# KaffinPX/neptune-core

Measured on AMD Instinct MI355X. Metric: STARK proofs verified/sec (whole node) + Tip5 perms/sec vs VALU roofline, higher is better.
Workload: dtype u64 (Goldilocks mod p; XFE = cubic extension)

## Files before the change

neptune-core_amd/csrc/stark_kernels.hip:

```cpp
#include <hip/hip_ext.h>

#include <atomic>
#include <cstdlib>

#include "../../include/nhip_challenge_id.h"
#include "kernels.hpp"
#include "proof_codec.hpp"
#include "stark.hpp"
#include "tip5_device.hpp"
#include "xfe.hpp"

namespace nhip {

#ifndef NHIP_LAT_PRIO
#define NHIP_LAT_PRIO 2
#endif
__device__ __forceinline__ void latency_priority() {
    if constexpr (NHIP_LAT_PRIO > 0) __builtin_amdgcn_s_setprio(NHIP_LAT_PRIO);
}
static constexpr uint32_t AGE_PRIO_OLDEST = 2;
static constexpr uint32_t AGE_PRIO_MIN_PROOFS = 2048;
__device__ uint32_t g_batches_done;
struct AgePrio {
    uint32_t seq, k;
};
__device__ __forceinline__ void age_priority(AgePrio a, int base) {
    bool old = false;
    if (a.k) {
        const uint32_t done = __builtin_amdgcn_readfirstlane(
            __hip_atomic_load(&g_batches_done, __ATOMIC_RELAXED, __HIP_MEMORY_SCOPE_AGENT));
        old = (int32_t)(a.seq - done) < (int32_t)a.k;
    }
    switch (base + (old ? 1 : 0)) {
        case 0: break;
        case 1: __builtin_amdgcn_s_setprio(1); break;
        case 2: __builtin_amdgcn_s_setprio(2); break;
        default: __builtin_amdgcn_s_setprio(3); break;
    }
}
#ifndef NHIP_MP_PRIO
#define NHIP_MP_PRIO 1
#endif


template <bool MW>
__device__ __forceinline__ Xfe ld_xfe_w(const uint64_t* __restrict__ w, uint64_t off) {
    return {word_mont<MW>(w[off]), word_mont<MW>(w[off + 1]), word_mont<MW>(w[off + 2])};
}
__device__ __forceinline__ Xfe ld_xfe_raw(const uint64_t* __restrict__ w, uint64_t off) {
    return {w[off], w[off + 1], w[off + 2]};
}
__device__ __forceinline__ void st_xfe_raw(uint64_t* __restrict__ w, uint64_t off, Xfe v) {
    w[off] = v.c0;
    w[off + 1] = v.c1;
    w[off + 2] = v.c2;
}
__device__ __forceinline__ bool x_is_zero(Xfe a) { return (a.c0 | a.c1 | a.c2) == 0; }

__device__ __forceinline__ uint64_t root_of_unity(uint32_t log2n) {
    return b_pow(to_mont(7), (GL_P - 1) >> log2n);
}

template <bool MW>
__global__ void __launch_bounds__(64) k_decode(const uint64_t* __restrict__ words, const ProofIn* __restrict__ in,
                                               uint32_t n_proofs, Dims D, uint32_t fs_stride, uint32_t xs_stride,
                                               ProofDesc* __restrict__ desc, FsOp* __restrict__ ops,
                                               uint32_t* __restrict__ fail, unsigned long long* __restrict__ counters) {
    latency_priority();
    __shared__ ProofDesc spd;
    __shared__ uint32_t sfail;
    __shared__ int sdeg;
    const uint32_t p = blockIdx.x, lane = threadIdx.x;
    if (p >= n_proofs) return;
    const ProofIn pin = in[p];
    if (lane == 0) {
        uint64_t perms = 0, perms_lcw = 0;
        const ClaimLoc cl{pin.claim_off, pin.claim_in_n, pin.claim_out_n};
        uint32_t f = decode_stream<MW>(words, pin.off, pin.len, cl, D, spd, ops + (uint64_t)p * fs_stride, perms, perms_lcw);
        if (!f && spd.log2_ph != pin.sized_log2_ph) {
            f = FAIL_DECODE;
            spd = ProofDesc{};
            claim_offsets(spd, cl);
        }
        if (!f) {
            atomicAdd(counters + CNT_PERMS_STATIC, (unsigned long long)perms);
            atomicAdd(counters + CNT_PERMS_LCW, (unsigned long long)perms_lcw);
        }
        sfail = f;
        sdeg = -1;
    }
    __syncthreads();
    const uint32_t f = sfail;
    if (!f) {
        int deg = -1;
        for (uint32_t hi = spd.last_poly_n; hi > 0; hi = hi > 64 ? hi - 64 : 0) {
            bool nz = false;
            if (lane < hi) {
                const uint64_t* x = words + spd.last_poly_off + 3ull * (hi - 1 - lane);
                nz = (canon(x[0]) | canon(x[1]) | canon(x[2])) != 0;
            }
            const uint64_t b = __ballot(nz);
            if (b) {
                deg = (int)(hi - (uint32_t)__ffsll((unsigned long long)b));
                break;
            }
        }
        if (lane == 0) sdeg = deg;
    }
    __syncthreads();
    if (lane == 0) {
        if (!f) last_poly_finish(spd, sdeg, D);
        const SampleLayout sl = SampleLayout::of(D.d, spd.R);
        spd.fs_op_off = p * fs_stride;
        spd.xs_off = (uint64_t)p * xs_stride;
        spd.n_xs = f ? 0u : sl.total;
        spd.idx_off = (uint64_t)p * D.d.num_checks;
        fail[p] = f;
    }
    __syncthreads();
    const uint64_t* src = reinterpret_cast<const uint64_t*>(&spd);
    uint64_t* dst = reinterpret_cast<uint64_t*>(desc + p);
    for (uint32_t i = lane; i < sizeof(ProofDesc) / 8; i += 64) dst[i] = src[i];
}

template <bool PAIR, bool MW>
__device__ __forceinline__ void fs_replay_wide_body(uint32_t bx, const Tip5Lds& lds, const uint64_t* __restrict__ words,
                                                    const ProofDesc* __restrict__ desc,
                                                    const FsOp* __restrict__ ops, uint32_t n_proofs,
                                                    uint64_t* __restrict__ xs, uint32_t* __restrict__ idx_out,
                                                    const uint32_t* __restrict__ fail) {
    constexpr uint32_t LANES = PAIR ? 32u : 16u;
    const uint32_t e = threadIdx.x & 15u;
    const uint32_t h = PAIR ? (threadIdx.x >> 4) & 1u : 0u;
    const uint32_t g = (bx * blockDim.x + threadIdx.x) / LANES;
    if (g >= n_proofs || fail[g]) return;
    uint64_t rc[TIP5_ROUNDS];
#pragma unroll
    for (int r = 0; r < TIP5_ROUNDS; ++r) rc[r] = c_tip5_rc_raw[r * 16 + e];
    uint32_t cm[8];
#pragma unroll
    for (int j = 0; j < 8; ++j) cm[j] = h ? TIP5_MDS[j + 8] : TIP5_MDS[j];
    auto permute = [&](uint64_t st) {
        if constexpr (PAIR) return tip5_permute_pair(st, e, h, rc, cm, lds.lut);
        else return tip5_permute_wide<false>(st, e, rc, lds.lut);
    };
    const bool writer = h == 0;
    const ProofDesc& d = desc[g];
    uint64_t s = 0;
    uint64_t xcur = d.xs_off * 3;
    uint64_t icur = d.idx_off;
    const uint32_t row_shift = threadIdx.x & (64u - LANES);
    for (uint32_t o = 0; o < d.fs_op_n; ++o) {
        const FsOp op = ops[d.fs_op_off + o];
        if (op.kind == FS_ABSORB) {
            const uint64_t* __restrict__ src = words + op.arg;
            const uint32_t len = op.n;
            const uint32_t nchunks = len / TIP5_RATE + 1;
            uint64_t w = (e < TIP5_RATE && e < len) ? src[e] : 0ull;
// ... 941 lines not shown
        const Xfe except_last = x_sub(z, x_lift(w_inv));
        const Xfe zm1 = x_sub(z, x_one());
        Xfe zph = z;
        for (uint32_t q = 0; q < d.log2_ph; ++q) zph = x_mul(zph, zph);
        const Xfe cons = x_sub(zph, x_one());
        const bool z0 = x_is_zero(zm1), z1 = x_is_zero(cons), z3 = x_is_zero(except_last);
        if (z0 || z1 || z3) zero_flag = 1u;
        const Xfe a = z0 ? x_one() : zm1, b = z1 ? x_one() : cons, c = z3 ? x_one() : except_last;
        const Xfe ab = x_mul(a, b);
        const Xfe iabc = x_inv(x_mul(ab, c));
        const Xfe iab = x_mul(iabc, c);
        const Xfe i1 = z1 ? x_zero() : x_mul(iab, a);
        zinv[0] = z0 ? x_zero() : x_mul(iab, b);
        zinv[1] = i1;
        zinv[2] = x_mul(except_last, i1);
        zinv[3] = z3 ? x_zero() : x_mul(iabc, ab);
    } else if (tid >= 64 && tid < 256) {
        auto chal = [&](uint32_t i) { return ld_xfe_raw(xs, xb + 3ull * (sl.chal + i)); };
        const uint32_t wv = tid >> 6;
        if (wv == 1) {
            const Xfe lut = eval_terminal_wave(256u, chal(CH_LOOKUP_TABLE_PUBLIC), [&](uint32_t i) {
                const uint64_t y = i + 1;
                return to_mont((y * y % 257u * y % 257u + 256u) % 257u);
            });
            if (tid == 64) chal_derived[2] = lut;
        } else if (wv == 2) {
            const Xfe ein = eval_terminal_wave(d.claim_in_n, chal(CH_STANDARD_INPUT),
                                               [&](uint32_t i) { return word_mont<MW>(words[d.claim_in_off + i]); });
            const Xfe comp = eval_terminal_wave(5u, chal(CH_COMPRESS_PROGRAM_DIGEST),
                                                [&](uint32_t i) { return word_mont<MW>(words[d.claim_digest_off + i]); });
            if (tid == 128) {
                chal_derived[0] = ein;
                chal_derived[3] = comp;
            }
        } else {
            const Xfe eout = eval_terminal_wave(d.claim_out_n, chal(CH_STANDARD_OUTPUT),
                                                [&](uint32_t i) { return word_mont<MW>(words[d.claim_out_off + i]); });
            if (tid == 192) chal_derived[1] = eout;
        }
    }
    __syncthreads();
    const uint32_t offs[5] = {0u, cons_type_off.x, cons_type_off.y, cons_type_off.z, cons_type_off.w};
    auto fetch = [&](uint32_t ref) -> Xfe {
        const uint32_t t = ref >> 30;
        if (t == 0) return slot_ld(ref);
        if (t == 1) return consts[ref & 0x3FFFFFFFu];
        const uint32_t kind = (ref >> 27) & 7u, i = ref & 0x7FFFFFFu;
        switch (kind) {
            case IN_MAIN_CURR: return ld_xfe_w<MW>(words, d.ood_mc + 3ull * i);
            case IN_AUX_CURR: return ld_xfe_w<MW>(words, d.ood_ac + 3ull * i);
            case IN_MAIN_NEXT: return ld_xfe_w<MW>(words, d.ood_mn + 3ull * i);
            case IN_AUX_NEXT: return ld_xfe_w<MW>(words, d.ood_an + 3ull * i);
            default:
                return i < dims.num_sampled ? ld_xfe_raw(xs, xb + 3ull * (sl.chal + i)) : chal_derived[i - dims.num_sampled];
        }
    };
    for (uint32_t lvl = 0; lvl < n_levels; ++lvl) {
        const uint32_t s0 = seg_off[3 * lvl], s1 = seg_off[3 * lvl + 1], s2 = seg_off[3 * lvl + 2],
                       s3 = seg_off[3 * lvl + 3];
        for (uint32_t q = s0 + tid; q < s1; q += blockDim.x) {
            const uint4 ins = reinterpret_cast<const uint4*>(prog)[q];
            slot_st(ins.w, fetch(ins.y));
        }
        for (uint32_t q = s1 + tid; q < s2; q += blockDim.x) {
            const uint4 ins = reinterpret_cast<const uint4*>(prog)[q];
            slot_st(ins.w, x_mul(slot_ld(ins.y), slot_ld(ins.z)));
        }
        for (uint32_t q = s2 + tid; q < s3; q += blockDim.x) {
            const uint4 ins = reinterpret_cast<const uint4*>(prog)[q];
            const Xfe x = slot_ld(ins.y), y = slot_ld(ins.z);
            slot_st(ins.w, ins.x == OOD_ADD ? x_add(x, y) : x_sub(x, y));
        }
        __syncthreads();
    }
    const uint32_t C = dims.num_constraints, cbase = lds_slots + gslot_n - C;
    Xfe acc = x_zero();
    for (uint32_t c = tid; c < C; c += blockDim.x) {
        uint32_t t = 0;
        while (t < 3 && c >= offs[t + 1]) ++t;
        const Xfe w = ld_xfe_raw(xs, xb + 3ull * (sl.quot_w + c));
        acc = x_add(acc, x_mul(w, x_mul(slot_ld(cbase + c), zinv[t])));
    }
    const Xfe ood_q = block_sum_xfe_waves(acc, red);
    const uint32_t M = dims.num_main, A = dims.num_aux, Q = dims.num_quot_seg;
    Xfe lc = x_zero(), ln = x_zero();
    for (uint32_t c = tid; c < M + A; c += blockDim.x) {
        const Xfe w = ld_xfe_raw(xs, xb + 3ull * (sl.lin_w + c));
        const Xfe vc = c < M ? ld_xfe_w<MW>(words, d.ood_mc + 3ull * c) : ld_xfe_w<MW>(words, d.ood_ac + 3ull * (c - M));
        const Xfe vn = c < M ? ld_xfe_w<MW>(words, d.ood_mn + 3ull * c) : ld_xfe_w<MW>(words, d.ood_an + 3ull * (c - M));
        lc = x_add(lc, x_mul(w, vc));
        ln = x_add(ln, x_mul(w, vn));
    }
    const Xfe sum_c = block_sum_xfe_waves(lc, red);
    const Xfe sum_n = block_sum_xfe_waves(ln, red);
    if (tid >= 64) return;
    Xfe seg = x_zero(), qlin = x_zero();
    for (uint32_t base = 0; base < Q; base += 64u) {
        const uint32_t q = base + tid, top = min(Q - 1u, base + 63u);
        Xfe zk = (q & 1u) ? z : x_one(), zp = z;
        for (uint32_t e = top >> 1, bit = 1; e; e >>= 1, ++bit) {
            zp = x_mul(zp, zp);
            zk = x_mul(zk, ((q >> bit) & 1u) ? zp : x_one());
        }
        if (q < Q) {
            const Xfe sq = ld_xfe_w<MW>(words, d.ood_qs + 3ull * q);
            seg = x_add(seg, x_mul(zk, sq));
            qlin = x_add(qlin, x_mul(ld_xfe_raw(xs, xb + 3ull * (sl.lin_w + M + A + q)), sq));
        }
    }
#pragma unroll
    for (int m = 32; m > 0; m >>= 1) {
        seg = x_add(seg, shfl_xor_xfe(seg, m));
        qlin = x_add(qlin, shfl_xor_xfe(qlin, m));
    }
    if (tid == 0) {
        uint32_t f = 0;
        if (zero_flag) f |= FAIL_ZERO_INVERSE;
        if (!x_eq(seg, ood_q)) f |= FAIL_OOD;
        if (f) atomicOr(&fail[p], f);
        uint64_t* o = ood_out + (uint64_t)p * 9;
        st_xfe_raw(o, 0, sum_c);
        st_xfe_raw(o, 3, sum_n);
        st_xfe_raw(o, 6, qlin);
    }
}

__device__ __forceinline__ uint64_t lds_pow(const uint64_t* __restrict__ sq, uint64_t e) {
    uint64_t r = MONT_ONE;
    for (uint32_t b = 0; e; ++b, e >>= 1)
        if (e & 1) r = mont_mul(r, sq[b]);
    return r;
}

#ifndef NHIP_FRI_WAVES
#define NHIP_FRI_WAVES 1
#endif
template <bool MW>
__device__ __forceinline__ void fri_body(uint32_t p, const uint64_t* __restrict__ words, const ProofDesc* __restrict__ desc,
                                         uint32_t n_proofs, StarkDims dims, const uint64_t* __restrict__ xs,
                                         const uint32_t* __restrict__ idx_all, uint64_t* __restrict__ xdom,
                                         uint32_t* __restrict__ fail) {
    __shared__ Xfe red[256];
    __shared__ uint64_t gsq[33], wsq[33];
    __shared__ uint32_t lflag;
    const uint32_t tid = threadIdx.x;
    if (p >= n_proofs || (fail[p] & FAIL_DECODE)) return;
    const ProofDesc& d = desc[p];
    const SampleLayout sl = SampleLayout::of(dims, d.R);
    const uint64_t xb = d.xs_off * 3;
    const uint32_t k = dims.num_checks;
    const uint32_t* __restrict__ idx = idx_all + d.idx_off;
    const uint32_t L = d.last_cw_n;
    const uint32_t log2L = 31 - __clz(L);
    if (tid == 0) {
        lflag = 0;
        uint64_t g = root_of_unity(d.log2_N);
        for (uint32_t q = 0; q < d.log2_N; ++q, g = mont_mul(g, g)) gsq[q] = g;
    } else if (tid == 64) {
        uint64_t w = root_of_unity(log2L);
        for (uint32_t q = 0; q < log2L; ++q, w = mont_mul(w, w)) wsq[q] = w;
    }
    __syncthreads();
    uint32_t f = 0;
    if (tid < k) {
        const uint32_t i0 = idx[tid];
        Xfe a = ld_xfe_w<MW>(words, d.fri[0].leaves_off + 3ull * tid);
        uint64_t x = mont_mul(to_mont(7), lds_pow(gsq, i0));
        xdom[(uint64_t)p * k + tid] = x;
        uint64_t xinv = b_inv(x);
        const uint64_t neg_half = to_mont((GL_P - 1) / 2);
        for (uint32_t r = 0; r < d.R; ++r) {
            const Xfe b = ld_xfe_w<MW>(words, d.fri[1 + r].leaves_off + 3ull * tid);
            const Xfe alpha = ld_xfe_raw(xs, xb + 3ull * (sl.alpha + r));
            const Xfe slope = x_scale(x_sub(b, a), mont_mul(neg_half, xinv));
            a = x_add(a, x_mul(slope, x_sub(alpha, x_lift(x))));
            x = mont_mul(x, x);
            xinv = mont_mul(xinv, xinv);
        }
        const Xfe last = ld_xfe_w<MW>(words, d.last_cw_off + 3ull * (i0 & (L - 1)));
        if (!x_eq(last, a)) f |= FAIL_FRI_LAST_AGREE;
    }
    const Xfe t = ld_xfe_raw(xs, xb + 3ull * sl.indeterminate);
    Xfe num = x_zero(), den = x_zero();
    if (tid < L) {
        uint64_t wi = lds_pow(wsq, tid);
        const uint64_t wstep = blockDim.x < L ? wsq[31 - __clz(blockDim.x)] : MONT_ONE;
        auto term = [&](uint32_t i, uint64_t w, Xfe inv) {
            const Xfe q = x_scale(inv, w);
            num = x_add(num, x_mul(q, ld_xfe_w<MW>(words, d.last_cw_off + 3ull * i)));
            den = x_add(den, q);
        };
        uint32_t i = tid;
        for (; i + blockDim.x < L; i += 2 * blockDim.x) {
            const uint64_t w1 = mont_mul(wi, wstep);
            const Xfe d0 = x_sub(t, x_lift(wi)), d1 = x_sub(t, x_lift(w1));
            const Xfe pr = x_mul(d0, d1);
            if (x_is_zero(pr)) {
                atomicOr(&lflag, 1u);
                term(i, wi, x_inv(d0));
                term(i + blockDim.x, w1, x_inv(d1));
            } else {
                const Xfe inv = x_inv(pr);
                term(i, wi, x_mul(inv, d1));
                term(i + blockDim.x, w1, x_mul(inv, d0));
            }
            wi = mont_mul(w1, wstep);
        }
        if (i < L) {
            const Xfe diff = x_sub(t, x_lift(wi));
            if (x_is_zero(diff)) atomicOr(&lflag, 1u);
            term(i, wi, x_inv(diff));
        }
    }
    const Xfe snum = block_sum_xfe(num, red);
    const Xfe sden = block_sum_xfe(den, red);
    __shared__ Xfe tpow[32];
    const uint32_t pbits = d.last_poly_n ? 32 - __clz(d.last_poly_n) : 0;
    if (tid == 0) {
        Xfe q = t;
        for (uint32_t j = 0; j < pbits; ++j, q = x_mul(q, q)) tpow[j] = q;
    }
    __syncthreads();
    Xfe hp = x_zero();
    for (uint32_t c = tid; c < d.last_poly_n; c += blockDim.x) {
        Xfe pw = x_one();
        for (uint32_t j = 0; (c >> j) != 0; ++j)
            if ((c >> j) & 1u) pw = x_mul(pw, tpow[j]);
        hp = x_add(hp, x_mul(pw, ld_xfe_w<MW>(words, d.last_poly_off + 3ull * c)));
    }
    const Xfe h = block_sum_xfe(hp, red);
    if (tid == 0) {
        if (lflag || x_is_zero(sden)) f |= FAIL_ZERO_INVERSE;
        else if (!x_eq(h, x_mul(snum, x_inv(sden)))) f |= FAIL_FRI_EVAL;
        if (!d.last_poly_degree_ok) f |= FAIL_FRI_DEGREE;
    }
    if (f) atomicOr(&fail[p], f);
}
template <bool MW>
__global__ void __launch_bounds__(256, NHIP_FRI_WAVES) k_fri(const uint64_t* __restrict__ words, const ProofDesc* __restrict__ desc,
                                             uint32_t n_proofs, StarkDims dims, const uint64_t* __restrict__ xs,
                                             const uint32_t* __restrict__ idx_all, uint64_t* __restrict__ xdom,
                                             uint32_t* __restrict__ fail) {
    latency_priority();
    fri_body<MW>(blockIdx.x, words, desc, n_proofs, dims, xs, idx_all, xdom, fail);
}

template <bool MW>
__global__ void __launch_bounds__(256) k_plan_fri_small(const uint64_t* __restrict__ words,
                                                        const ProofDesc* __restrict__ desc, uint32_t n_proofs,
                                                        uint32_t k, uint32_t trees_per_proof, uint32_t groups,
                                                        const uint64_t* __restrict__ dig,
                                                        const uint32_t* __restrict__ idx_all, MpPlan plan,
                                                        uint32_t* __restrict__ fail,
                                                        unsigned long long* __restrict__ perm_counter,
                                                        StarkDims dims, const uint64_t* __restrict__ xs,
                                                        uint64_t* __restrict__ xdom) {
    latency_priority();
    const uint32_t bx = blockIdx.x, np = n_proofs * groups;
    if (bx < np)
        mp_plan_body<256>(bx % n_proofs, bx / n_proofs, words, desc, n_proofs, k, trees_per_proof, dig, idx_all, plan,
                          fail, perm_counter);
    else
        fri_body<MW>(bx - np, words, desc, n_proofs, dims, xs, idx_all, xdom, fail);
}

typedef unsigned __int128 u128_t;
static constexpr uint32_t DEEP_UNROLL = 8;

__device__ __forceinline__ uint64_t reduce_u108(u128_t y) {
    const uint64_t y0 = (uint64_t)y, y1 = (uint64_t)(y >> 64);
    const uint64_t r = reduce96(y0, (uint32_t)y1);
    return gl_sub(r, y1 >> 32);
}

__device__ __forceinline__ uint64_t shfl_xor_u64(uint64_t v, int m) {
    return (uint64_t)__shfl_xor((long long)v, m);
}

__device__ __forceinline__ uint4 w_limbs(uint64_t w) {
    return make_uint4((uint32_t)w & 0x3FFFFFu, (uint32_t)(w >> 22) & 0x3FFFFFu, (uint32_t)(w >> 44), 0u);
}
__device__ __forceinline__ void wl_mac(uint64_t (&a)[6], uint4 wl, uint32_t x0, uint32_t x1) {
    a[0] += (uint64_t)wl.x * x0;
    a[1] += (uint64_t)wl.y * x0;
    a[2] += (uint64_t)wl.z * x0;
    a[3] += (uint64_t)wl.x * x1;
    a[4] += (uint64_t)wl.y * x1;
    a[5] += (uint64_t)wl.z * x1;
}
__device__ __forceinline__ uint64_t wl_reduce(const uint64_t (&a)[6]) {
    const u128_t U = (u128_t)a[0] + ((u128_t)a[1] << 22) + ((u128_t)a[2] << 44);
    const u128_t W = (u128_t)a[3] + ((u128_t)a[4] << 22) + ((u128_t)a[5] << 44);
    const uint64_t ur = reduce_u108(U), wr = reduce_u108(W);
    return gl_add(ur, reduce96(wr << 32, (uint32_t)(wr >> 32)));
}

#ifndef NHIP_DEEP_WAVES
#define NHIP_DEEP_WAVES 6
#endif
template <bool MW>
__global__ void __launch_bounds__(256, NHIP_DEEP_WAVES) k_deep_rows8(const uint64_t* __restrict__ words,
                                                    const ProofDesc* __restrict__ desc, uint32_t n_proofs,
                                                    StarkDims dims, const uint64_t* __restrict__ xs,
                                                    const uint64_t* __restrict__ xdom,
                                                    const uint64_t* __restrict__ ood, uint32_t* __restrict__ fail) {
    extern __shared__ __attribute__((aligned(16))) unsigned char smem[];
    const uint32_t M = dims.num_main, A = dims.num_aux, Q = dims.num_quot_seg, k = dims.num_checks;
    uint4* wm = reinterpret_cast<uint4*>(smem);
    uint4* wa = wm + 3 * M;
    Xfe* rowsum = reinterpret_cast<Xfe*>(wa + 9 * A);
    __shared__ Xfe s_quot[MAX_CHECKS];
    __shared__ Xfe s_at[3];
    const uint32_t p = blockIdx.x, tid = threadIdx.x;
    if (p >= n_proofs || (fail[p] & FAIL_DECODE)) return;
    const ProofDesc& d = desc[p];
    const SampleLayout sl = SampleLayout::of(dims, d.R);
    const uint64_t xb = d.xs_off * 3;
    const uint64_t* __restrict__ lw = xs + xb + 3ull * sl.lin_w;
    for (uint32_t i = tid; i < 3 * M; i += blockDim.x) wm[i] = w_limbs(lw[i]);
    for (uint32_t c = tid; c < A; c += blockDim.x) {
        const uint64_t w0 = lw[3 * (M + c)], w1 = lw[3 * (M + c) + 1], w2 = lw[3 * (M + c) + 2];
        uint4* o = wa + 9 * c;
        o[0] = w_limbs(w0), o[1] = w_limbs(w1), o[2] = w_limbs(w2);
        o[3] = w_limbs(gl_sub(0, w2)), o[4] = w_limbs(gl_add(w0, w2)), o[5] = w_limbs(w1);
        o[6] = w_limbs(gl_sub(0, w1)), o[7] = w_limbs(gl_sub(w1, w2)), o[8] = w_limbs(gl_add(w0, w2));
    }
    if (tid == blockDim.x - 1) {
        const Xfe z = ld_xfe_raw(xs, xb + 3ull * sl.z);
        s_at[0] = z;
        s_at[1] = x_scale(z, root_of_unity(d.log2_ph));
        Xfe zq = x_one();
        for (uint32_t q = 0; q < Q; ++q) zq = x_mul(zq, z);
        s_at[2] = zq;
    }
    __syncthreads();
    const uint32_t q8 = tid & 7u, rloc = tid >> 3;
    const uint32_t rows_per_pass = blockDim.x >> 3;
    for (uint32_t j0 = 0; j0 < k; j0 += rows_per_pass) {
        const uint32_t j = j0 + rloc;
        uint64_t acc[3][6];
#pragma unroll
        for (int c = 0; c < 3; ++c)
#pragma unroll
            for (int q = 0; q < 6; ++q) acc[c][q] = 0;
        if (j < k) {
            const uint64_t* __restrict__ mrow = words + d.main_rows_off + (uint64_t)j * M;
            uint32_t c = q8;
            for (; c + 8 * (DEEP_UNROLL - 1) < M; c += 8 * DEEP_UNROLL) {
                uint64_t xv[DEEP_UNROLL];
#pragma unroll
                for (uint32_t u = 0; u < DEEP_UNROLL; ++u) xv[u] = mrow[c + 8 * u];
#pragma unroll
                for (uint32_t u = 0; u < DEEP_UNROLL; ++u) {
                    const uint32_t cc = c + 8 * u, x0 = (uint32_t)xv[u], x1 = (uint32_t)(xv[u] >> 32);
                    wl_mac(acc[0], wm[3 * cc], x0, x1);
                    wl_mac(acc[1], wm[3 * cc + 1], x0, x1);
                    wl_mac(acc[2], wm[3 * cc + 2], x0, x1);
                }
            }
            for (; c < M; c += 8) {
                const uint64_t xw = mrow[c];
                const uint32_t x0 = (uint32_t)xw, x1 = (uint32_t)(xw >> 32);
                wl_mac(acc[0], wm[3 * c], x0, x1);
                wl_mac(acc[1], wm[3 * c + 1], x0, x1);
                wl_mac(acc[2], wm[3 * c + 2], x0, x1);
            }
            const uint64_t* __restrict__ arow = words + d.aux_rows_off + (uint64_t)j * 3 * A;
            const uint32_t WA = 3 * A;
            uint32_t w = q8;
            for (; w + 8 * (DEEP_UNROLL - 1) < WA; w += 8 * DEEP_UNROLL) {
                uint64_t xv[DEEP_UNROLL];
#pragma unroll
                for (uint32_t u = 0; u < DEEP_UNROLL; ++u) xv[u] = arow[w + 8 * u];
#pragma unroll
                for (uint32_t u = 0; u < DEEP_UNROLL; ++u) {
                    const uint4* wt = wa + 3 * (w + 8 * u);
                    const uint32_t x0 = (uint32_t)xv[u], x1 = (uint32_t)(xv[u] >> 32);
                    wl_mac(acc[0], wt[0], x0, x1);
                    wl_mac(acc[1], wt[1], x0, x1);
                    wl_mac(acc[2], wt[2], x0, x1);
                }
            }
            for (; w < WA; w += 8) {
                const uint4* wt = wa + 3 * w;
                const uint64_t xw = arow[w];
                const uint32_t x0 = (uint32_t)xw, x1 = (uint32_t)(xw >> 32);
                wl_mac(acc[0], wt[0], x0, x1);
                wl_mac(acc[1], wt[1], x0, x1);
                wl_mac(acc[2], wt[2], x0, x1);
            }
        }
        uint64_t v0 = wl_reduce(acc[0]), v1 = wl_reduce(acc[1]), v2 = wl_reduce(acc[2]);
#pragma unroll
        for (int m = 1; m < 8; m <<= 1) {
            v0 = gl_add(v0, shfl_xor_u64(v0, m));
            v1 = gl_add(v1, shfl_xor_u64(v1, m));
            v2 = gl_add(v2, shfl_xor_u64(v2, m));
        }
        if (j < k && q8 == 0) {
            if constexpr (MW) rowsum[j] = {from_mont(v0), from_mont(v1), from_mont(v2)};
            else rowsum[j] = {v0, v1, v2};
        }
        if (j < k && q8 == 1) {
            Xfe qv = x_zero();
            for (uint32_t q = 0; q < Q; ++q)
                qv = x_add(qv, x_mul(ld_xfe_raw(lw, 3ull * (M + A + q)),
                                     ld_xfe_raw(words, d.quot_rows_off + (uint64_t)j * 3 * Q + 3ull * q)));
            if constexpr (MW) s_quot[j] = qv;
            else s_quot[j] = {to_mont(qv.c0), to_mont(qv.c1), to_mont(qv.c2)};
        }
    }
    __syncthreads();
    uint32_t f = 0;
    for (uint32_t j2 = tid; j2 < k; j2 += blockDim.x) {
        const Xfe row = rowsum[j2];
        const Xfe x = x_lift(xdom[(uint64_t)p * k + j2]);
        const Xfe d0 = x_sub(x, s_at[0]), d1 = x_sub(x, s_at[1]), d2 = x_sub(x, s_at[2]);
        const Xfe d01 = x_mul(d0, d1);
        const Xfe prod = x_mul(d01, d2);
        if (x_is_zero(prod)) {
            f |= FAIL_ZERO_INVERSE;
            continue;
        }
        const Xfe inv = x_inv(prod);
        const Xfe inv2 = x_mul(inv, d01);
        const Xfe inv01 = x_mul(inv, d2);
        const Xfe inv0 = x_mul(inv01, d1);
        const Xfe inv1 = x_mul(inv01, d0);
        const uint64_t* __restrict__ oo = ood + (uint64_t)p * 9;
        const uint64_t* __restrict__ wd = lw + 3ull * (M + A + Q);
        const Xfe t0 = x_mul(x_mul(x_sub(row, ld_xfe_raw(oo, 0)), inv0), ld_xfe_raw(wd, 0));
        const Xfe t1 = x_mul(x_mul(x_sub(row, ld_xfe_raw(oo, 3)), inv1), ld_xfe_raw(wd, 3));
        const Xfe t2 = x_mul(x_mul(x_sub(s_quot[j2], ld_xfe_raw(oo, 6)), inv2), ld_xfe_raw(wd, 6));
        const Xfe deep = x_add(x_add(t0, t1), t2);
        const Xfe fri_v = ld_xfe_w<MW>(words, d.fri[0].leaves_off + 3ull * j2);
        if (!x_eq(deep, fri_v)) f |= FAIL_DEEP;
    }
    if (f) atomicOr(&fail[p], f);
}

__global__ void k_verdicts(const uint32_t* __restrict__ fail, uint32_t n, uint8_t* __restrict__ v) {
    const uint32_t i = blockIdx.x * blockDim.x + threadIdx.x;
    if (i < n) v[i] = fail[i] == 0 ? 1 : 0;
    if (i == 0) atomicAdd(&g_batches_done, 1u);
}
static constexpr uint32_t ROOTS_ONE_WG = 1024;
template <bool MW>
__global__ void __launch_bounds__(ROOTS_ONE_WG) k_roots_verdicts_small(
    const uint64_t* __restrict__ words, const ProofDesc* __restrict__ desc, const uint64_t* __restrict__ dig,
    MpPlan plan, uint32_t n_records, uint32_t trees_per_proof, uint32_t k, uint32_t* __restrict__ fail,
    uint32_t n_proofs, LcwTree lcw, uint8_t* __restrict__ v) {
    const uint32_t i = threadIdx.x;
    mp_roots_body<MW>(i, words, desc, dig, plan, n_records, trees_per_proof, k, fail, n_proofs, lcw);
    __threadfence();
    __syncthreads();
    if (i < n_proofs) v[i] = __hip_atomic_load(&fail[i], __ATOMIC_RELAXED, __HIP_MEMORY_SCOPE_AGENT) == 0 ? 1 : 0;
    if (i == 0) atomicAdd(&g_batches_done, 1u);
}

template <typename K, typename... A>
static void launch_ev(K kernel, dim3 grid, dim3 block, size_t shm, hipStream_t s, hipEvent_t e0, hipEvent_t e1,
                      A... args) {
    if (e0 || e1) hipExtLaunchKernelGGL(kernel, grid, block, shm, s, e0, e1, 0, args...);
    else hipLaunchKernelGGL(kernel, grid, block, shm, s, args...);
}

static bool ood_wide(uint32_t n) {
    static const uint32_t lim = [] {
        const char* v = nhip::ab_env("NHIP_OOD_WIDE_MAX");
        return v ? (uint32_t)std::strtoul(v, nullptr, 10) : OOD_WIDE_MAX_PROOFS;
    }();
    return n <= lim;
}

static constexpr uint32_t CLIMB_FROM_MIN_LEVELS = 24;
static constexpr uint64_t CLIMB_FROM_OPS_DEFAULT = 4096;
static std::atomic<int64_t>& climb_from_forced() {
    static std::atomic<int64_t> v(-1);
    return v;
}
int set_climb_from_ops(int64_t ops) {
    if (ops < -1) return -1;
    climb_from_forced().store(ops, std::memory_order_relaxed);
    return 0;
}
static uint64_t climb_from_ops(uint32_t hash_levels) {
    const int64_t v = climb_from_forced().load(std::memory_order_relaxed);
    if (v >= 0) return (uint64_t)v;
    return hash_levels >= CLIMB_FROM_MIN_LEVELS ? CLIMB_FROM_OPS_DEFAULT : 0ull;
}


static constexpr uint32_t ROWS_WIDE_MAX_PROOFS = 32;
static uint32_t rows_wide_max() {
    static const uint32_t v = [] {
        const char* e = nhip::ab_env("NHIP_ROWS_WIDE_MAX");
        return e ? (uint32_t)std::strtoul(e, nullptr, 10) : ROWS_WIDE_MAX_PROOFS;
    }();
    return v;
}

enum FsForm { FS_ROW = 0, FS_PAIR = 1, FS_QUAD = 2 };
static uint32_t quad_wg() {
    static const uint32_t v = [] {
        const char* e = nhip::ab_env("NHIP_QUAD_WG");
        const uint32_t w = e ? (uint32_t)std::strtoul(e, nullptr, 10) : FS_QUAD_WG;
        return (w >= 64 && w <= 1024 && w % 64 == 0) ? w : FS_QUAD_WG;
    }();
    return v;
}
static std::atomic<int>& fs_form_forced() {
    static std::atomic<int> f([] {
        if (const char* v = nhip::ab_env("NHIP_FS_FORM")) {
            if (v[0] == 'q') return (int)FS_QUAD;
            if (v[0] == 'p') return (int)FS_PAIR;
            if (v[0] == 'r') return (int)FS_ROW;
        }
        return -1;
    }());
    return f;
}
int set_fs_form(int form) {
    if (form < -1 || form > (int)FS_QUAD) return -1;
    fs_form_forced().store(form, std::memory_order_relaxed);
    return 0;
}
static FsForm fs_form(uint32_t n) {
    static const uint32_t quad_min = [] {
        const char* v = nhip::ab_env("NHIP_FS_QUAD_MIN");
        return v ? (uint32_t)std::strtoul(v, nullptr, 10) : FS_QUAD_MIN_PROOFS;
    }();
    const int forced = fs_form_forced().load(std::memory_order_relaxed);
    if (forced >= 0) return (FsForm)forced;
    if (n < FS_PAIR_MAX_PROOFS) return FS_PAIR;
    return n >= quad_min ? FS_QUAD : FS_ROW;
}

#ifdef NHIP_AB_BUILD
__global__ void k_pad_packet() {}
#endif

template <bool MW>
static hipError_t launch_phases(const StarkBatchDev& b, hipStream_t st, hipStream_t sa, StarkPhaseTimer* tm) {
    const uint32_t n = b.n_proofs;
    if (n == 0) return hipSuccess;
    (void)hipGetLastError();
    const uint32_t k = b.dims.num_checks;
    const uint32_t tpp = 4 + b.max_R;
    const bool two = st != sa;
    constexpr uint32_t SYNC = (1u << 12) | (1u << 0) | (1u << 1) | (1u << 3) | (1u << 7) | (1u << 10) | (1u << 8);
    auto mark = [&](int i, hipStream_t s) {
        if (tm->phase_marks || (two && ((SYNC >> i) & 1u))) (void)hipEventRecord(tm->ev[i], s);
    };
    auto wait = [&](hipStream_t s, int i) {
        if (two) (void)hipStreamWaitEvent(s, tm->ev[i], 0);
    };
#ifdef NHIP_AB_BUILD
    static const int pad_n = [] {
        const char* e = nhip::ab_env("NHIP_PAD_PACKETS");
        return e ? std::atoi(e) : 0;
    }();
    auto pad = [&](hipStream_t s) {
        for (int i = 0; i < pad_n; ++i) hipLaunchKernelGGL(k_pad_packet, dim3(1), dim3(64), 0, s);
    };
#else
    auto pad = [](hipStream_t) {};
#endif
    const bool small = n <= climb_max_proofs();
    static const int64_t age_env = [] {
        const char* e = nhip::ab_env("NHIP_AGE_PRIO");
        return e ? (int64_t)std::strtoul(e, nullptr, 10) : (int64_t)-1;
    }();
    const uint32_t age_k = age_env >= 0 ? (uint32_t)age_env : (n >= AGE_PRIO_MIN_PROOFS ? AGE_PRIO_OLDEST : 0u);
    static std::atomic<uint32_t> seq_ctr[64];
    int dev = 0;
    (void)hipGetDevice(&dev);
    const AgePrio age{seq_ctr[(uint32_t)dev & 63u].fetch_add(1u, std::memory_order_relaxed), age_k};
    static const bool age_fs = [] {
        const char* e = nhip::ab_env("NHIP_AGE_PRIO_FS");
        return e && e[0] == '1';
    }();
    const AgePrio age_sponge{age.seq, age_fs ? age.k : 0u};
    mark(12, st);
    wait(sa, 12);
    hipLaunchKernelGGL(k_decode<MW>, dim3(n), dim3(64), 0, sa, b.words, b.in, n, b.D, b.fs_stride, b.xs_stride, b.desc,
                       b.ops, b.fail, b.counters);
// ... 208 lines not shown
```

neptune-core_amd/csrc/xfe.hpp:

```cpp
#pragma once
#include "goldilocks.hpp"

namespace nhip {

struct Xfe {
    uint64_t c0, c1, c2;
};

static constexpr uint64_t MONT_ONE_W = 0x00000000FFFFFFFFull;

__host__ __device__ __forceinline__ Xfe x_zero() { return {0, 0, 0}; }
__host__ __device__ __forceinline__ Xfe x_one() { return {MONT_ONE_W, 0, 0}; }
__host__ __device__ __forceinline__ Xfe x_lift(uint64_t b) { return {b, 0, 0}; }

__host__ __device__ __forceinline__ Xfe x_add(Xfe a, Xfe b) {
    return {gl_add(a.c0, b.c0), gl_add(a.c1, b.c1), gl_add(a.c2, b.c2)};
}
__host__ __device__ __forceinline__ Xfe x_sub(Xfe a, Xfe b) {
    return {gl_sub(a.c0, b.c0), gl_sub(a.c1, b.c1), gl_sub(a.c2, b.c2)};
}
__host__ __device__ __forceinline__ Xfe x_scale(Xfe a, uint64_t s) {
    return {mont_mul(a.c0, s), mont_mul(a.c1, s), mont_mul(a.c2, s)};
}
__host__ __device__ __forceinline__ bool x_eq(Xfe a, Xfe b) { return a.c0 == b.c0 && a.c1 == b.c1 && a.c2 == b.c2; }

struct U128 {
    uint64_t lo, hi;
};
struct U160 {
    uint64_t lo, hi;
    uint32_t top;
};

__host__ __device__ __forceinline__ U128 mul128(uint64_t a, uint64_t b) {
    const uint32_t a0 = (uint32_t)a, a1 = (uint32_t)(a >> 32);
    const uint32_t b0 = (uint32_t)b, b1 = (uint32_t)(b >> 32);
    const uint64_t p00 = (uint64_t)a0 * b0;
    const uint64_t t = (uint64_t)a0 * b1 + (p00 >> 32);
    const uint64_t u = (uint64_t)a1 * b0 + (uint32_t)t;
    const uint64_t v = (uint64_t)a1 * b1 + (t >> 32);
    return {(u << 32) | (uint32_t)p00, v + (u >> 32)};
}

__host__ __device__ __forceinline__ U160 add160(U160 x, U128 y) {
    unsigned int c0, c1, c2, c3;
    const uint32_t l0 = __builtin_addc((uint32_t)x.lo, (uint32_t)y.lo, 0u, &c0);
    const uint32_t l1 = __builtin_addc((uint32_t)(x.lo >> 32), (uint32_t)(y.lo >> 32), c0, &c1);
    const uint32_t h0 = __builtin_addc((uint32_t)x.hi, (uint32_t)y.hi, c1, &c2);
    const uint32_t h1 = __builtin_addc((uint32_t)(x.hi >> 32), (uint32_t)(y.hi >> 32), c2, &c3);
    return {((uint64_t)l1 << 32) | l0, ((uint64_t)h1 << 32) | h0, x.top + c3};
}
__host__ __device__ __forceinline__ U160 wide(U128 x) { return {x.lo, x.hi, 0u}; }

__host__ __device__ __forceinline__ U160 sub160_2p(U160 x, U160 y) {
    unsigned int c0, c1, b0, b1, b2, b3;
    const uint32_t h0 = __builtin_addc((uint32_t)x.hi, 2u, 0u, &c0);
    const uint32_t h1 = __builtin_addc((uint32_t)(x.hi >> 32), 0xFFFFFFFEu, c0, &c1);
    const uint32_t l0 = __builtin_subc((uint32_t)x.lo, (uint32_t)y.lo, 0u, &b0);
    const uint32_t l1 = __builtin_subc((uint32_t)(x.lo >> 32), (uint32_t)(y.lo >> 32), b0, &b1);
    const uint32_t g0 = __builtin_subc(h0, (uint32_t)y.hi, b1, &b2);
    const uint32_t g1 = __builtin_subc(h1, (uint32_t)(y.hi >> 32), b2, &b3);
    return {((uint64_t)l1 << 32) | l0, ((uint64_t)g1 << 32) | g0, x.top + 1u + c1 - y.top - b3};
}

__host__ __device__ __forceinline__ uint64_t red160(U160 x) {
    const uint64_t tt = ((uint64_t)x.top << 32) - x.top;
    uint64_t h = x.hi + tt;
    if (h < tt) h += GL_EPS;
    const uint32_t xl0 = (uint32_t)x.lo, xl1 = (uint32_t)(x.lo >> 32);
    unsigned int e, br1, br2, c1, c, c2;
    const uint32_t ah = __builtin_addc(xl1, xl0, 0u, &e);
    const uint32_t bl = __builtin_subc(xl0, ah, e, &br1);
    const uint32_t bh = __builtin_subc(ah, 0u, br1, &br2);
    uint32_t rl = __builtin_subc((uint32_t)h, bl, 0u, &c1);
    uint32_t rh = __builtin_subc((uint32_t)(h >> 32), bh, c1, &c);
    const uint32_t m = 0u - c;
    rl = __builtin_subc(rl, m, 0u, &c2);
    rh = rh - c2;
    const uint64_t r = ((uint64_t)rh << 32) | rl;
    return r >= GL_P ? r - GL_P : r;
}

__host__ __device__ __forceinline__ Xfe x_mul(Xfe a, Xfe b) {
    const U128 p12 = mul128(a.c1, b.c2), p21 = mul128(a.c2, b.c1), p00 = mul128(a.c0, b.c0);
    const U160 n = add160(wide(p12), p21);
    Xfe r;
    r.c0 = red160(sub160_2p(wide(p00), n));
    const U128 p01 = mul128(a.c0, b.c1), p10 = mul128(a.c1, b.c0), p22 = mul128(a.c2, b.c2);
    U160 s1 = add160(add160(wide(p01), p10), U128{n.lo, n.hi});
    s1.top += n.top;
    r.c1 = red160(sub160_2p(s1, wide(p22)));
    const U128 p02 = mul128(a.c0, b.c2), p11 = mul128(a.c1, b.c1), p20 = mul128(a.c2, b.c0);
    r.c2 = red160(add160(add160(add160(wide(p02), p11), p20), p22));
    return r;
}

__host__ __device__ __forceinline__ uint64_t b_sqn(uint64_t x, int n) {
#pragma unroll 1
    for (int i = 0; i < n; ++i) x = mont_mul(x, x);
    return x;
}

__host__ __device__ __forceinline__ uint64_t b_inv(uint64_t a) {
    const uint64_t t2 = mont_mul(mont_mul(a, a), a);
    const uint64_t t3 = mont_mul(mont_mul(t2, t2), a);
    const uint64_t t6 = mont_mul(b_sqn(t3, 3), t3);
    const uint64_t t12 = mont_mul(b_sqn(t6, 6), t6);
    const uint64_t t15 = mont_mul(b_sqn(t12, 3), t3);
    const uint64_t t30 = mont_mul(b_sqn(t15, 15), t15);
    const uint64_t t31 = mont_mul(mont_mul(t30, t30), a);
    const uint64_t t32m2 = mont_mul(t31, t31);
    const uint64_t t32 = mont_mul(t32m2, a);
    return mont_mul(b_sqn(t32m2, 32), t32);
}

__host__ __device__ __forceinline__ uint64_t b_pow(uint64_t a, uint64_t e) {
    uint64_t r = MONT_ONE_W;
    while (e) {
        if (e & 1) r = mont_mul(r, a);
        a = mont_mul(a, a);
        e >>= 1;
    }
    return r;
}

__host__ __device__ __forceinline__ Xfe x_inv(Xfe a) {
    const uint64_t s = gl_add(a.c0, a.c2);
    const uint64_t d = gl_sub(a.c1, a.c2);
    const uint64_t C00 = gl_sub(mont_mul(s, s), mont_mul(d, a.c1));
    const uint64_t C01 = gl_sub(mont_mul(d, a.c2), mont_mul(a.c1, s));
    const uint64_t C02 = gl_sub(mont_mul(a.c1, a.c1), mont_mul(s, a.c2));
    const uint64_t det = gl_sub(gl_sub(mont_mul(a.c0, C00), mont_mul(a.c2, C01)), mont_mul(a.c1, C02));
    const uint64_t di = b_inv(det);
    return {mont_mul(C00, di), mont_mul(C01, di), mont_mul(C02, di)};
}

__host__ __device__ __forceinline__ Xfe x_pow(Xfe a, uint64_t e) {
    Xfe r = x_one();
    while (e) {
        if (e & 1) r = x_mul(r, a);
        a = x_mul(a, a);
        e >>= 1;
    }
    return r;
}

}
```

Before: 469,500.

## Batch base-field inversions across workgroup and replace per-point inverses with table lookups

Adds a workgroup-wide Montgomery batch inversion (wave prefix/suffix products plus one b_inv per block) and uses it for the last-codeword barycentric denominators and for the DEEP quotient denominators. The FRI x^-1 is now computed from the precomputed power table using the inverse exponent, and the root-of-unity ladders are filled in parallel from a constant table instead of by a serial squaring loop. In the DEEP kernel the quotient-row combination moves from the row pass into the per-check loop, which frees the shared s_quot buffer. In exchange the code adds extra __syncthreads and shuffle-scan work per iteration, and the quotient sum now runs on one thread per check instead of being spread across lanes.

Result: no change. 472,500, median of 6 (+0.6%).

```diff
diff --git a/neptune-core_amd/csrc/batch_inv.hpp b/neptune-core_amd/csrc/batch_inv.hpp
--- /dev/null
+++ b/neptune-core_amd/csrc/batch_inv.hpp
@@ -0,0 +1,44 @@
+#pragma once
+#include "xfe.hpp"
+
+namespace nhip {
+
+static constexpr uint32_t WG_BINV_LDS_WORDS = 17;
+
+__device__ __forceinline__ uint64_t wg_batch_inv(uint64_t v, bool live, uint64_t* __restrict__ sh) {
+    const uint32_t lane = threadIdx.x & 63u, nw = blockDim.x >> 6;
+    const uint32_t wv = __builtin_amdgcn_readfirstlane(threadIdx.x >> 6);
+    const bool use = live && v != 0;
+    const bool any = __ballot(use) != 0;
+    uint64_t pre = use ? v : MONT_ONE_W, suf = pre;
+    if (any) {
+#pragma unroll
+        for (uint32_t m = 1; m < 64; m <<= 1) {
+            const uint64_t up = (uint64_t)__shfl_up((long long)pre, m);
+            const uint64_t dn = (uint64_t)__shfl_down((long long)suf, m);
+            pre = mont_mul(pre, lane >= m ? up : MONT_ONE_W);
+            suf = mont_mul(suf, lane + m < 64u ? dn : MONT_ONE_W);
+        }
+    }
+    if (lane == 63u) sh[wv] = pre;
+    __syncthreads();
+    if (wv == 0) {
+        uint64_t t = sh[0];
+        for (uint32_t w = 1; w < nw; ++w) t = mont_mul(t, sh[w]);
+        const uint64_t ti = b_inv(t);
+        if (lane == 0) sh[nw] = ti;
+    }
+    __syncthreads();
+    uint64_t o = sh[nw];
+    if (any)
+        for (uint32_t w = 0; w < nw; ++w)
+            if (w != wv) o = mont_mul(o, sh[w]);
+    __syncthreads();
+    if (!any) return 0;
+    const uint64_t bp = (uint64_t)__shfl_up((long long)pre, 1u), bs = (uint64_t)__shfl_down((long long)suf, 1u);
+    const uint64_t before = lane ? bp : MONT_ONE_W, after = lane < 63u ? bs : MONT_ONE_W;
+    const uint64_t r = mont_mul(mont_mul(before, after), o);
+    return use ? r : 0;
+}
+
+}
diff --git a/neptune-core_amd/csrc/stark_kernels.hip b/neptune-core_amd/csrc/stark_kernels.hip
--- a/neptune-core_amd/csrc/stark_kernels.hip
+++ b/neptune-core_amd/csrc/stark_kernels.hip
@@ -4,6 +4,7 @@
 #include <cstdlib>
 
 #include "../../include/nhip_challenge_id.h"
+#include "batch_inv.hpp"
 #include "kernels.hpp"
 #include "proof_codec.hpp"
 #include "stark.hpp"
@@ -1251,14 +1252,9 @@
     const uint32_t* __restrict__ idx = idx_all + d.idx_off;
     const uint32_t L = d.last_cw_n;
     const uint32_t log2L = 31 - __clz(L);
-    if (tid == 0) {
-        lflag = 0;
-        uint64_t g = root_of_unity(d.log2_N);
-        for (uint32_t q = 0; q < d.log2_N; ++q, g = mont_mul(g, g)) gsq[q] = g;
-    } else if (tid == 64) {
-        uint64_t w = root_of_unity(log2L);
-        for (uint32_t q = 0; q < log2L; ++q, w = mont_mul(w, w)) wsq[q] = w;
-    }
+    if (tid == 0) lflag = 0;
+    if (tid < d.log2_N) gsq[tid] = gl_root_of_unity(d.log2_N - tid);
+    else if (tid >= 64 && tid - 64 < log2L) wsq[tid - 64] = gl_root_of_unity(log2L - (tid - 64));
     __syncthreads();
     uint32_t f = 0;
     if (tid < k) {
@@ -1266,7 +1262,7 @@
         Xfe a = ld_xfe_w<MW>(words, d.fri[0].leaves_off + 3ull * tid);
         uint64_t x = mont_mul(to_mont(7), lds_pow(gsq, i0));
         xdom[(uint64_t)p * k + tid] = x;
-        uint64_t xinv = b_inv(x);
+        uint64_t xinv = coset_point_inv(gsq, d.log2_N, i0);
         const uint64_t neg_half = to_mont((GL_P - 1) / 2);
         for (uint32_t r = 0; r < d.R; ++r) {
             const Xfe b = ld_xfe_w<MW>(words, d.fri[1 + r].leaves_off + 3ull * tid);
@@ -1281,34 +1277,34 @@
     }
     const Xfe t = ld_xfe_raw(xs, xb + 3ull * sl.indeterminate);
     Xfe num = x_zero(), den = x_zero();
-    if (tid < L) {
-        uint64_t wi = lds_pow(wsq, tid);
+    {
+        uint64_t wi = tid < L ? lds_pow(wsq, tid) : MONT_ONE;
         const uint64_t wstep = blockDim.x < L ? wsq[31 - __clz(blockDim.x)] : MONT_ONE;
         auto term = [&](uint32_t i, uint64_t w, Xfe inv) {
             const Xfe q = x_scale(inv, w);
             num = x_add(num, x_mul(q, ld_xfe_w<MW>(words, d.last_cw_off + 3ull * i)));
             den = x_add(den, q);
         };
-        uint32_t i = tid;
-        for (; i + blockDim.x < L; i += 2 * blockDim.x) {
+        for (uint32_t i0 = 0; i0 < L; i0 += 2 * blockDim.x) {
+            const uint32_t i = i0 + tid;
+            const bool one = i < L, two = i + blockDim.x < L;
             const uint64_t w1 = mont_mul(wi, wstep);
             const Xfe d0 = x_sub(t, x_lift(wi)), d1 = x_sub(t, x_lift(w1));
-            const Xfe pr = x_mul(d0, d1);
-            if (x_is_zero(pr)) {
-                atomicOr(&lflag, 1u);
-                term(i, wi, x_inv(d0));
-                term(i + blockDim.x, w1, x_inv(d1));
-            } else {
-                const Xfe inv = x_inv(pr);
-                term(i, wi, x_mul(inv, d1));
-                term(i + blockDim.x, w1, x_mul(inv, d0));
+            const Xfe pr = two ? x_mul(d0, d1) : d0;
+            if (one && x_is_zero(pr)) atomicOr(&lflag, 1u);
+            uint64_t det;
+            const Xfe adj = x_adj_det(pr, det);
+            const uint64_t di = wg_batch_inv(det, one, reinterpret_cast<uint64_t*>(red));
+            if (one) {
+                const Xfe inv = x_scale(adj, di);
+                if (two) {
+                    term(i, wi, x_mul(inv, d1));
+                    term(i + blockDim.x, w1, x_mul(inv, d0));
+                } else {
+                    term(i, wi, inv);
+                }
             }
             wi = mont_mul(w1, wstep);
-        }
-        if (i < L) {
-            const Xfe diff = x_sub(t, x_lift(wi));
-            if (x_is_zero(diff)) atomicOr(&lflag, 1u);
-            term(i, wi, x_inv(diff));
         }
     }
     const Xfe snum = block_sum_xfe(num, red);
@@ -1408,7 +1404,7 @@
     uint4* wm = reinterpret_cast<uint4*>(smem);
     uint4* wa = wm + 3 * M;
     Xfe* rowsum = reinterpret_cast<Xfe*>(wa + 9 * A);
-    __shared__ Xfe s_quot[MAX_CHECKS];
+    __shared__ uint64_t s_binv[WG_BINV_LDS_WORDS];
     __shared__ Xfe s_at[3];
     const uint32_t p = blockIdx.x, tid = threadIdx.x;
     if (p >= n_proofs || (fail[p] & FAIL_DECODE)) return;
@@ -1427,7 +1423,7 @@
     if (tid == blockDim.x - 1) {
         const Xfe z = ld_xfe_raw(xs, xb + 3ull * sl.z);
         s_at[0] = z;
-        s_at[1] = x_scale(z, root_of_unity(d.log2_ph));
+        s_at[1] = x_scale(z, gl_root_of_unity(d.log2_ph));
         Xfe zq = x_one();
         for (uint32_t q = 0; q < Q; ++q) zq = x_mul(zq, z);
         s_at[2] = zq;
@@ -1500,28 +1496,28 @@
             if constexpr (MW) rowsum[j] = {from_mont(v0), from_mont(v1), from_mont(v2)};
             else rowsum[j] = {v0, v1, v2};
         }
-        if (j < k && q8 == 1) {
-            Xfe qv = x_zero();
-            for (uint32_t q = 0; q < Q; ++q)
-                qv = x_add(qv, x_mul(ld_xfe_raw(lw, 3ull * (M + A + q)),
-                                     ld_xfe_raw(words, d.quot_rows_off + (uint64_t)j * 3 * Q + 3ull * q)));
-            if constexpr (MW) s_quot[j] = qv;
-            else s_quot[j] = {to_mont(qv.c0), to_mont(qv.c1), to_mont(qv.c2)};
-        }
     }
     __syncthreads();
     uint32_t f = 0;
-    for (uint32_t j2 = tid; j2 < k; j2 += blockDim.x) {
-        const Xfe row = rowsum[j2];
-        const Xfe x = x_lift(xdom[(uint64_t)p * k + j2]);
-        const Xfe d0 = x_sub(x, s_at[0]), d1 = x_sub(x, s_at[1]), d2 = x_sub(x, s_at[2]);
-        const Xfe d01 = x_mul(d0, d1);
-        const Xfe prod = x_mul(d01, d2);
-        if (x_is_zero(prod)) {
+    for (uint32_t jb = 0; jb < k; jb += blockDim.x) {
+        const uint32_t j2 = jb + tid;
+        const bool live = j2 < k;
+        Xfe d0 = x_zero(), d1 = x_zero(), d2 = x_zero(), d01 = x_zero(), adj = x_zero();
+        uint64_t det = 0;
+        if (live) {
+            const Xfe x = x_lift(xdom[(uint64_t)p * k + j2]);
+            d0 = x_sub(x, s_at[0]), d1 = x_sub(x, s_at[1]), d2 = x_sub(x, s_at[2]);
+            d01 = x_mul(d0, d1);
+            adj = x_adj_det(x_mul(d01, d2), det);
+        }
+        const uint64_t di = wg_batch_inv(det, live, s_binv);
+        if (!live) continue;
+        if (det == 0) {
             f |= FAIL_ZERO_INVERSE;
             continue;
         }
-        const Xfe inv = x_inv(prod);
+        const Xfe row = rowsum[j2];
+        const Xfe inv = x_scale(adj, di);
         const Xfe inv2 = x_mul(inv, d01);
         const Xfe inv01 = x_mul(inv, d2);
         const Xfe inv0 = x_mul(inv01, d1);
@@ -1530,7 +1526,12 @@
         const uint64_t* __restrict__ wd = lw + 3ull * (M + A + Q);
         const Xfe t0 = x_mul(x_mul(x_sub(row, ld_xfe_raw(oo, 0)), inv0), ld_xfe_raw(wd, 0));
         const Xfe t1 = x_mul(x_mul(x_sub(row, ld_xfe_raw(oo, 3)), inv1), ld_xfe_raw(wd, 3));
-        const Xfe t2 = x_mul(x_mul(x_sub(s_quot[j2], ld_xfe_raw(oo, 6)), inv2), ld_xfe_raw(wd, 6));
+        Xfe qv = x_zero();
+        for (uint32_t q = 0; q < Q; ++q)
+            qv = x_add(qv, x_mul(ld_xfe_raw(lw, 3ull * (M + A + q)),
+                                 ld_xfe_raw(words, d.quot_rows_off + (uint64_t)j2 * 3 * Q + 3ull * q)));
+        if constexpr (!MW) qv = {to_mont(qv.c0), to_mont(qv.c1), to_mont(qv.c2)};
+        const Xfe t2 = x_mul(x_mul(x_sub(qv, ld_xfe_raw(oo, 6)), inv2), ld_xfe_raw(wd, 6));
         const Xfe deep = x_add(x_add(t0, t1), t2);
         const Xfe fri_v = ld_xfe_w<MW>(words, d.fri[0].leaves_off + 3ull * j2);
         if (!x_eq(deep, fri_v)) f |= FAIL_DEEP;
diff --git a/neptune-core_amd/csrc/xfe.hpp b/neptune-core_amd/csrc/xfe.hpp
--- a/neptune-core_amd/csrc/xfe.hpp
+++ b/neptune-core_amd/csrc/xfe.hpp
@@ -124,15 +124,46 @@
     return r;
 }
 
-__host__ __device__ __forceinline__ Xfe x_inv(Xfe a) {
+__host__ __device__ __forceinline__ uint64_t gl_root_of_unity(uint32_t k) {
+    constexpr uint64_t T[33] = {
+        0x00000000FFFFFFFFull, 0xFFFFFFFE00000002ull, 0xFFFFFFFEFFFF0001ull, 0xFEFFFFFF01000001ull,
+        0x0000000010000000ull, 0xFFFFBFFF00000001ull, 0xFFFFFFFEFFFFFF81ull, 0x07FFFFFFFFFFF800ull,
+        0xE60CA9645A7A425Eull, 0x5C411F4D8AB91088ull, 0x8BFED970D671FBB7ull, 0x1DA1C8CEDC0A82B1ull,
+        0x959DFCB4779EB1B1ull, 0x35D17996B4E99746ull, 0x10BBA1E10E56548Bull, 0x2306BAAAE6467556ull,
+        0xBF79450CEBA724C2ull, 0xAA3D8A0CA9F1CF0Aull, 0x05F9BEAB78DE26D9ull, 0x8CAA33007781B093ull,
+        0x5E93E76C70B1E9C6ull, 0x32322652D8CB2AB7ull, 0xE67246B3CE63A09Eull, 0x36FBC989DE66DC62ull,
+        0xC307E16FB62A525Eull, 0x6ECFEFD745751A91ull, 0x78D6E28499E74D1Full, 0x915A171C5DCE5B0Bull,
+        0x004A4484A6B1267Bull, 0xA46D26647BEA105Full, 0xB86A0843C8FA27B2ull, 0x5588E6586A6C9A32ull,
+        0xDA58878B0D514E98ull};
+    return T[k];
+}
+
+__host__ __device__ __forceinline__ Xfe x_adj_det(Xfe a, uint64_t& det) {
     const uint64_t s = gl_add(a.c0, a.c2);
     const uint64_t d = gl_sub(a.c1, a.c2);
     const uint64_t C00 = gl_sub(mont_mul(s, s), mont_mul(d, a.c1));
     const uint64_t C01 = gl_sub(mont_mul(d, a.c2), mont_mul(a.c1, s));
     const uint64_t C02 = gl_sub(mont_mul(a.c1, a.c1), mont_mul(s, a.c2));
-    const uint64_t det = gl_sub(gl_sub(mont_mul(a.c0, C00), mont_mul(a.c2, C01)), mont_mul(a.c1, C02));
-    const uint64_t di = b_inv(det);
-    return {mont_mul(C00, di), mont_mul(C01, di), mont_mul(C02, di)};
+    det = gl_sub(gl_sub(mont_mul(a.c0, C00), mont_mul(a.c2, C01)), mont_mul(a.c1, C02));
+    return {C00, C01, C02};
+}
+
+__host__ __device__ __forceinline__ Xfe x_inv(Xfe a) {
+    uint64_t det;
+    const Xfe adj = x_adj_det(a, det);
+    return x_scale(adj, b_inv(det));
+}
+
+static constexpr uint64_t GL_INV7 = (GL_P + 1) / 7;
+static_assert((GL_P + 1) % 7 == 0, "7^-1 mod p");
+__host__ __device__ __forceinline__ uint64_t coset_point_inv(const uint64_t* __restrict__ sq, uint32_t log2n,
+                                                             uint64_t i) {
+    const uint64_t mask = ((uint64_t)1 << log2n) - 1;
+    uint64_t e = (mask + 1 - i) & mask;
+    uint64_t r = to_mont(GL_INV7);
+    for (uint32_t b = 0; e; ++b, e >>= 1)
+        if (e & 1) r = mont_mul(r, sq[b]);
+    return r;
 }
 
 __host__ __device__ __forceinline__ Xfe x_pow(Xfe a, uint64_t e) {
```
